# RKWin93/E2E-MAPPO-for-MT-FJSP

Hardware: NVIDIA B200
Metric: MT-FJSP env-steps/sec (higher is better)
Workload: dtype f64

## Files before the change

### e2e-mappo-for-mt-fjsp_b200/csrc/mtfjsp_gemm.cu

```cuda
#include <cuda.h>
#include <cuda_runtime.h>
#include <stdint.h>
#include <stdlib.h>

#include <type_traits>

#include "../../include/mtfjsp.h"

namespace {

constexpr int TILE_M = 128, TILE_N = 128;

__device__ __forceinline__ uint32_t smem_u32(const void* p) { return (uint32_t)__cvta_generic_to_shared(p); }
__device__ __forceinline__ float to_tf32(float x) {
    uint32_t r;
    asm("cvt.rna.tf32.f32 %0, %1;" : "=r"(r) : "f"(x));
    return __uint_as_float(r);
}
__device__ __forceinline__ void mbar_init(uint32_t bar, uint32_t count) {
    asm volatile("mbarrier.init.shared::cta.b64 [%0], %1;" ::"r"(bar), "r"(count));
}
__device__ __forceinline__ void mbar_wait(uint32_t bar, uint32_t parity) {
    uint32_t ok;
    do {
        asm volatile(
            "{\n\t.reg .pred p;\n\t"
            "mbarrier.try_wait.parity.shared::cta.b64 p, [%1], %2;\n\t"
            "selp.u32 %0, 1, 0, p;\n\t}"
            : "=r"(ok)
            : "r"(bar), "r"(parity)
            : "memory");
    } while (!ok);
}
__device__ __forceinline__ uint64_t make_desc(uint32_t saddr, uint32_t lbo_bytes, uint32_t sbo_bytes) {
    uint64_t d = 0;
    d |= (uint64_t)((saddr & 0x3FFFF) >> 4);
    d |= (uint64_t)(lbo_bytes >> 4) << 16;
    d |= (uint64_t)(sbo_bytes >> 4) << 32;
    d |= 1ull << 46;
    return d;
}
constexpr uint32_t IDESC = (1u << 4) | (2u << 7) | (2u << 10) | ((TILE_N >> 3) << 17) | ((TILE_M >> 4) << 24);

__device__ __forceinline__ void umma_tf32(uint32_t tmem_d, uint64_t adesc, uint64_t bdesc, uint32_t accumulate) {
    asm volatile(
        "{\n\t.reg .pred p;\n\tsetp.ne.b32 p, %4, 0;\n\t"
        "tcgen05.mma.cta_group::1.kind::tf32 [%0], %1, %2, %3, p;\n\t}" ::"r"(tmem_d),
        "l"(adesc), "l"(bdesc), "r"(IDESC), "r"(accumulate));
}

#define TMEM_LD32(taddr, r)                                                                                          \
    asm volatile(                                                                                                    \
        "tcgen05.ld.sync.aligned.32x32b.x32.b32 "                                                                    \
        "{%0,%1,%2,%3,%4,%5,%6,%7,%8,%9,%10,%11,%12,%13,%14,%15,%16,%17,%18,%19,%20,%21,%22,%23,%24,%25,%26,%27,%28,"  \
        "%29,%30,%31}, [%32];"                                                                                       \
        : "=r"(r[0]), "=r"(r[1]), "=r"(r[2]), "=r"(r[3]), "=r"(r[4]), "=r"(r[5]), "=r"(r[6]), "=r"(r[7]), "=r"(r[8]),  \
          "=r"(r[9]), "=r"(r[10]), "=r"(r[11]), "=r"(r[12]), "=r"(r[13]), "=r"(r[14]), "=r"(r[15]), "=r"(r[16]),       \
          "=r"(r[17]), "=r"(r[18]), "=r"(r[19]), "=r"(r[20]), "=r"(r[21]), "=r"(r[22]), "=r"(r[23]), "=r"(r[24]),      \
          "=r"(r[25]), "=r"(r[26]), "=r"(r[27]), "=r"(r[28]), "=r"(r[29]), "=r"(r[30]), "=r"(r[31])                    \
        : "r"(taddr))

template <bool AFFINE, int NWARPS>
__device__ __forceinline__ void stage_block(float* sdst, const float* __restrict__ g, long long row0, long long rows,
                                            int K, int KP, int ld, const float* s_scale, const float* s_shift,
                                            bool relu, int warp, int lane) {
    const int sbo = (KP / 4) * 128;
    const int r = lane & 7, c = lane >> 3;
    const int quads = KP / 16;
    const int total = 16 * quads;
    constexpr int U = 8;
    for (int it0 = warp; it0 < total; it0 += NWARPS * U) {
        float4 v[U];
#pragma unroll
        for (int u = 0; u < U; u++) {
            const int it = it0 + u * NWARPS;
            const int grp = it / quads, q = it - grp * quads;
            const long long row = row0 + grp * 8 + r;
            const int k = q * 16 + c * 4;
            v[u] = make_float4(0.f, 0.f, 0.f, 0.f);
            if (it < total && row < rows && k < K) v[u] = __ldg(reinterpret_cast<const float4*>(g + row * ld + k));
        }
#pragma unroll
        for (int u = 0; u < U; u++) {
            const int it = it0 + u * NWARPS;
            if (it >= total) break;
            const int grp = it / quads, q = it - grp * quads;
            const long long row = row0 + grp * 8 + r;
            const int k = q * 16 + c * 4;
            float4 x = v[u];
            if (AFFINE) {
                if (row < rows && k < K) {
                    x.x = x.x * s_scale[k] + s_shift[k]; x.y = x.y * s_scale[k + 1] + s_shift[k + 1];
                    x.z = x.z * s_scale[k + 2] + s_shift[k + 2]; x.w = x.w * s_scale[k + 3] + s_shift[k + 3];
                    if (relu) { x.x = fmaxf(x.x, 0.f); x.y = fmaxf(x.y, 0.f); x.z = fmaxf(x.z, 0.f); x.w = fmaxf(x.w, 0.f); }
                }
            }
            x.x = to_tf32(x.x); x.y = to_tf32(x.y); x.z = to_tf32(x.z); x.w = to_tf32(x.w);
            *reinterpret_cast<float4*>(reinterpret_cast<char*>(sdst) + grp * sbo + (q * 4 + c) * 128 + r * 16) = x;
        }
    }
}

constexpr int NPROD = 8;

template <int KS>
__device__ __forceinline__ void tile_issue(float* sdst, const float* __restrict__ g, long long row0, long long rows, int K,
                                           int kbase, int pw, int lane) {
    constexpr int SBO = (KS / 4) * 128, QUADS = KS / 16, TOTAL = 16 * QUADS;
    const int r = lane & 7, c = lane >> 3;
    static_assert(NPROD % QUADS == 0, "a warp keeps one K chunk: its folded BatchNorm constants live in registers");
#pragma unroll
    for (int it = pw; it < TOTAL; it += NPROD) {
        const int grp = it / QUADS, q = it % QUADS;
// ... 755 lines not shown
        for (int c = 0; c < nparts; c++) t += parts[((size_t)c * TILE_M + m) * NP + k];
        dW[idx] = t;
    }
    if (db && idx < TILE_M) {
        float t = 0.f;
        for (int c = 0; c < nparts; c++) t += dbparts[(size_t)c * 128 + idx];
        db[idx] = t;
    }
}


__device__ __forceinline__ float tanh_fast(float x) {
    const float t = __expf(2.f * fminf(x, 44.f));
    return 1.f - __fdividef(2.f, t + 1.f);
}
__device__ __forceinline__ float elu_fast(float x) { return x > 0.f ? x : __expf(x) - 1.f; }

constexpr int HEAD_WARPS = 16;

template <bool GROUPED>
__global__ void __launch_bounds__(HEAD_WARPS * 32, 1) head_tf32_kernel(
    const float* __restrict__ X, const int32_t* __restrict__ cand, long long rows, int rpe, int nodes_per_env,
    const float* __restrict__ in_scale, const float* __restrict__ in_shift, int in_relu, const float* __restrict__ Wa,
    const float* __restrict__ bias_env, long long bias_rows, const float* __restrict__ W1, const float* __restrict__ b1,
    const float* __restrict__ w2, const float* __restrict__ b2, float* __restrict__ out, long long num_tiles, int epg = 1) {
    extern __shared__ __align__(1024) unsigned char smem[];
    constexpr size_t WBYTES = (size_t)TILE_N * 128 * 4;
    float* sWa = reinterpret_cast<float*>(smem);
    float* sW1 = reinterpret_cast<float*>(smem + WBYTES);
    float* sA = reinterpret_cast<float*>(smem + 2 * WBYTES);
    float* s_part = reinterpret_cast<float*>(smem + 3 * WBYTES);
    float* s_b1 = s_part + 4 * 128;
    float* s_w2 = s_b1 + 128;
    float* s_scale = s_w2 + 128;
    float* s_shift = s_scale + 128;
    int* s_row = reinterpret_cast<int*>(s_shift + 128);
    uint64_t* s_bar = reinterpret_cast<uint64_t*>(s_row + 256);
    uint32_t* s_tmem = reinterpret_cast<uint32_t*>(s_bar + 2);

    const int tid = threadIdx.x, warp = tid >> 5, lane = tid & 31;
    const bool affine = in_scale != nullptr;
    if (tid < 128) {
        s_b1[tid] = b1 ? b1[tid] : 0.f;
        s_w2[tid] = w2[tid];
        s_scale[tid] = affine ? in_scale[tid] : 1.f;
        s_shift[tid] = affine ? in_shift[tid] : 0.f;
    }
    if (tid == 0) {
        mbar_init(smem_u32(s_bar + 0), 1);
        mbar_init(smem_u32(s_bar + 1), 1);
        asm volatile("fence.mbarrier_init.release.cluster;" ::: "memory");
    }
    if (warp == 0) {
        asm volatile("tcgen05.alloc.cta_group::1.sync.aligned.shared::cta.b32 [%0], %1;" ::"r"(smem_u32(s_tmem)), "r"(256));
        asm volatile("tcgen05.relinquish_alloc_permit.cta_group::1.sync.aligned;");
    }
    stage_block<false, HEAD_WARPS>(sWa, Wa, 0, TILE_N, 128, 128, 128, nullptr, nullptr, false, warp, lane);
    stage_block<false, HEAD_WARPS>(sW1, W1, 0, TILE_N, 128, 128, 128, nullptr, nullptr, false, warp, lane);
    auto fill_rows = [&](long long tile, int slot) {
        const long long r = tile * TILE_M + tid;
        int src = -1;
        if (tile < num_tiles && r < rows) src = cand ? (int)((r / rpe) * nodes_per_env + __ldg(cand + r)) : (int)r;
        s_row[slot * 128 + tid] = src;
    };
    if (tid < 128) fill_rows(blockIdx.x, 0);
    asm volatile("fence.proxy.async.shared::cta;" ::: "memory");
    asm volatile("tcgen05.fence::before_thread_sync;" ::: "memory");
    __syncthreads();
    asm volatile("tcgen05.fence::after_thread_sync;" ::: "memory");
    const uint32_t tmem_base = *s_tmem;
    const uint32_t bar0 = smem_u32(s_bar), bar1 = smem_u32(s_bar + 1);
    const float b2v = b2 ? __ldg(b2) : 0.f;

    const int r8 = lane & 7, c4 = lane >> 3;
    float4 v[8];
    auto gather = [&](int slot) {
#pragma unroll
        for (int u = 0; u < 8; u++) {
            const int it = warp + u * HEAD_WARPS, grp = it >> 3, q = it & 7;
            const int src = s_row[slot * 128 + grp * 8 + r8];
            v[u] = src >= 0 ? __ldg(reinterpret_cast<const float4*>(X + (size_t)src * 128 + q * 16 + c4 * 4)) : make_float4(0.f, 0.f, 0.f, 0.f);
        }
    };
    auto store_a = [&](int slot) {
#pragma unroll
        for (int u = 0; u < 8; u++) {
            const int it = warp + u * HEAD_WARPS, grp = it >> 3, q = it & 7, k = q * 16 + c4 * 4;
            float4 x = v[u];
            if (affine && s_row[slot * 128 + grp * 8 + r8] >= 0) {
                float4 sc, sh;
                if (GROUPED) {
                    const int src = s_row[slot * 128 + grp * 8 + r8];
                    const long long g = (long long)(cand ? src / nodes_per_env : src / rpe) / epg;
                    sc = __ldg(reinterpret_cast<const float4*>(in_scale + g * 128 + k));
                    sh = __ldg(reinterpret_cast<const float4*>(in_shift + g * 128 + k));
                } else {
                    sc = *reinterpret_cast<const float4*>(s_scale + k); sh = *reinterpret_cast<const float4*>(s_shift + k);
                }
                x.x = x.x * sc.x + sh.x; x.y = x.y * sc.y + sh.y; x.z = x.z * sc.z + sh.z; x.w = x.w * sc.w + sh.w;
                if (in_relu) { x.x = fmaxf(x.x, 0.f); x.y = fmaxf(x.y, 0.f); x.z = fmaxf(x.z, 0.f); x.w = fmaxf(x.w, 0.f); }
            }
            x.x = to_tf32(x.x); x.y = to_tf32(x.y); x.z = to_tf32(x.z); x.w = to_tf32(x.w);
            *reinterpret_cast<float4*>(reinterpret_cast<char*>(sA) + grp * 4096 + (q * 4 + c4) * 128 + r8 * 16) = x;
        }
    };
    auto mma_tile = [&](const float* sW, uint32_t dcol) {
        asm volatile("tcgen05.fence::after_thread_sync;" ::: "memory");
        const uint32_t aA = smem_u32(sA), aW = smem_u32(sW);
#pragma unroll
        for (int k = 0; k < 16; k++)
            umma_tf32(tmem_base + dcol, make_desc(aA + k * 256, 128, 4096), make_desc(aW + k * 256, 128, 4096), k > 0 ? 1u : 0u);
    };

    const int quad = warp & 3, cg = warp >> 2;
    const int trow = quad * 32 + lane;
    gather(0);
    long long i = 0;
    for (long long tile = blockIdx.x; tile < num_tiles; tile += gridDim.x, i++) {
        const int slot = (int)(i & 1);
        const uint32_t par = (uint32_t)(i & 1);
        store_a(slot);
        if (tid < 128) fill_rows(tile + gridDim.x, slot ^ 1);
        asm volatile("fence.proxy.async.shared::cta;" ::: "memory");
        asm volatile("tcgen05.fence::before_thread_sync;" ::: "memory");
        __syncthreads();
        if (tid == 0) {
            mma_tile(sWa, 0);
            asm volatile("tcgen05.commit.cta_group::1.mbarrier::arrive::one.shared::cluster.b64 [%0];" ::"r"(bar0) : "memory");
        }
        gather(slot ^ 1);
        mbar_wait(bar0, par);
        asm volatile("tcgen05.fence::after_thread_sync;" ::: "memory");
        const long long grow = tile * TILE_M + trow;
        const bool rok = grow < rows;
        {
            uint32_t r[32];
            TMEM_LD32(tmem_base + ((uint32_t)(quad * 32) << 16) + (uint32_t)(cg * 32), r);
            asm volatile("tcgen05.wait::ld.sync.aligned;" ::: "memory");
            const long long brow = bias_rows == 1 ? 0 : (rok ? grow / rpe : 0);
            const float4* bp = reinterpret_cast<const float4*>(bias_env + brow * 128 + cg * 32);
            char* dst = reinterpret_cast<char*>(sA) + (trow >> 3) * 4096 + (cg * 8) * 128 + (trow & 7) * 16;
#pragma unroll
            for (int j = 0; j < 8; j++) {
                const float4 bb = __ldg(bp + j);
                float4 x;
                x.x = to_tf32(tanh_fast(__uint_as_float(r[4 * j]) + bb.x)); x.y = to_tf32(tanh_fast(__uint_as_float(r[4 * j + 1]) + bb.y));
                x.z = to_tf32(tanh_fast(__uint_as_float(r[4 * j + 2]) + bb.z)); x.w = to_tf32(tanh_fast(__uint_as_float(r[4 * j + 3]) + bb.w));
                if (!rok) x = make_float4(0.f, 0.f, 0.f, 0.f);
                *reinterpret_cast<float4*>(dst + j * 128) = x;
            }
        }
        asm volatile("fence.proxy.async.shared::cta;" ::: "memory");
        asm volatile("tcgen05.fence::before_thread_sync;" ::: "memory");
        __syncthreads();
        if (tid == 0) {
            mma_tile(sW1, TILE_N);
            asm volatile("tcgen05.commit.cta_group::1.mbarrier::arrive::one.shared::cluster.b64 [%0];" ::"r"(bar1) : "memory");
        }
        mbar_wait(bar1, par);
        asm volatile("tcgen05.fence::after_thread_sync;" ::: "memory");
        {
            uint32_t r[32];
            TMEM_LD32(tmem_base + ((uint32_t)(quad * 32) << 16) + (uint32_t)(TILE_N + cg * 32), r);
            asm volatile("tcgen05.wait::ld.sync.aligned;" ::: "memory");
            float acc = 0.f;
#pragma unroll
            for (int j = 0; j < 8; j++) {
                const float4 bb = *reinterpret_cast<const float4*>(s_b1 + cg * 32 + 4 * j);
                const float4 ww = *reinterpret_cast<const float4*>(s_w2 + cg * 32 + 4 * j);
                acc = fmaf(tanh_fast(__uint_as_float(r[4 * j]) + bb.x), ww.x, acc);
                acc = fmaf(tanh_fast(__uint_as_float(r[4 * j + 1]) + bb.y), ww.y, acc);
                acc = fmaf(tanh_fast(__uint_as_float(r[4 * j + 2]) + bb.z), ww.z, acc);
                acc = fmaf(tanh_fast(__uint_as_float(r[4 * j + 3]) + bb.w), ww.w, acc);
            }
            s_part[cg * 128 + trow] = acc;
        }
        asm volatile("tcgen05.fence::before_thread_sync;" ::: "memory");
        __syncthreads();
        if (tid < 128) {
            const long long orow = tile * TILE_M + tid;
            if (orow < rows) out[orow] = ((s_part[tid] + s_part[128 + tid]) + (s_part[256 + tid] + s_part[384 + tid])) + b2v;
        }
    }
    asm volatile("tcgen05.fence::before_thread_sync;" ::: "memory");
    __syncthreads();
    if (warp == 0) asm volatile("tcgen05.dealloc.cta_group::1.sync.aligned.b32 %0, %1;" ::"r"(tmem_base), "r"(256));
}


constexpr int TRUNK_WARPS = 16;
template <bool GROUPED>
__global__ void __launch_bounds__(TRUNK_WARPS * 32, 1) gat_trunk2_tf32_kernel(
    const float* __restrict__ f1, const float* __restrict__ f2, const float* __restrict__ W1p, const float* __restrict__ W2p,
    const float* __restrict__ Wt, const float* __restrict__ a_src, const float* __restrict__ a_dst, float* __restrict__ out,
    double* __restrict__ stats, long long R, long long num_tiles, int rpt, int M) {
    extern __shared__ __align__(1024) unsigned char smem[];
    constexpr size_t WBYTES = (size_t)TILE_N * 128 * 4;
    float* sW = reinterpret_cast<float*>(smem);
    float* sA1 = reinterpret_cast<float*>(smem + WBYTES);
    float* sA2 = reinterpret_cast<float*>(smem + 2 * WBYTES);
    float* s_dot = reinterpret_cast<float*>(smem + 3 * WBYTES);
    float* s_as = s_dot + 3 * 4 * 128;
    float* s_ad = s_as + 128;
    float* s_w1p = s_ad + 128;
    float* s_w2p = s_w1p + 128 * 6;
    uint64_t* s_bar = reinterpret_cast<uint64_t*>(s_w2p + 128 * 8);
    uint32_t* s_tmem = reinterpret_cast<uint32_t*>(s_bar + 1);

    const int tid = threadIdx.x, warp = tid >> 5, lane = tid & 31;
    if (tid < 128) { s_as[tid] = a_src[tid]; s_ad[tid] = a_dst[tid]; }
    for (int i = tid; i < 128 * 6; i += blockDim.x) s_w1p[i] = W1p[i];
    for (int i = tid; i < 128 * 8; i += blockDim.x) s_w2p[i] = W2p[i];
    if (tid == 0) {
        mbar_init(smem_u32(s_bar), 1);
        asm volatile("fence.mbarrier_init.release.cluster;" ::: "memory");
    }
    if (warp == 0) {
        asm volatile("tcgen05.alloc.cta_group::1.sync.aligned.shared::cta.b32 [%0], %1;" ::"r"(smem_u32(s_tmem)), "r"(256));
        asm volatile("tcgen05.relinquish_alloc_permit.cta_group::1.sync.aligned;");
    }
    stage_block<false, TRUNK_WARPS>(sW, Wt, 0, TILE_N, 128, 128, 128, nullptr, nullptr, false, warp, lane);
    asm volatile("fence.proxy.async.shared::cta;" ::: "memory");
    asm volatile("tcgen05.fence::before_thread_sync;" ::: "memory");
    __syncthreads();
    asm volatile("tcgen05.fence::after_thread_sync;" ::: "memory");
    const uint32_t tmem_base = *s_tmem;
    const uint32_t bar = smem_u32(s_bar);

    const int quad = warp & 3, cg = warp >> 2;
    const int mloc = quad * 32 + lane;
    const size_t arow = (size_t)(mloc >> 3) * 4096 + (cg * 8) * 128 + (mloc & 7) * 16;
    uint32_t phase = 0;
    double st_sum = 0.0, st_sq = 0.0;
    for (long long tile = blockIdx.x; tile < num_tiles; tile += gridDim.x) {
        const long long m = tile * (GROUPED ? rpt : 128) + mloc;
        const bool mok = m < R && (!GROUPED || mloc < rpt);
        {
            float fa[6] = {0.f, 0.f, 0.f, 0.f, 0.f, 0.f}, fb[8] = {0.f, 0.f, 0.f, 0.f, 0.f, 0.f, 0.f, 0.f};
            if (mok) {
                const float2* p2 = reinterpret_cast<const float2*>(f1 + m * 6);
                const float2 u0 = __ldg(p2), u1 = __ldg(p2 + 1), u2 = __ldg(p2 + 2);
                fa[0] = u0.x; fa[1] = u0.y; fa[2] = u1.x; fa[3] = u1.y; fa[4] = u2.x; fa[5] = u2.y;
                const float4 v0 = __ldg(reinterpret_cast<const float4*>(f2 + m * 8)), v1 = __ldg(reinterpret_cast<const float4*>(f2 + m * 8) + 1);
                fb[0] = v0.x; fb[1] = v0.y; fb[2] = v0.z; fb[3] = v0.w; fb[4] = v1.x; fb[5] = v1.y; fb[6] = v1.z; fb[7] = v1.w;
            }
#pragma unroll
            for (int j = 0; j < 8; j++) {
                float o1[4], o2[4];
// ... 23 lines not shown
                for (int k = 0; k < 16; k++)
                    umma_tf32(tmem_base, make_desc(a1 + k * 256, 128, 4096), make_desc(aW + k * 256, 128, 4096), k > 0 ? 1u : 0u);
#pragma unroll
                for (int k = 0; k < 16; k++)
                    umma_tf32(tmem_base + TILE_N, make_desc(a2 + k * 256, 128, 4096), make_desc(aW + k * 256, 128, 4096), k > 0 ? 1u : 0u);
                asm volatile("tcgen05.commit.cta_group::1.mbarrier::arrive::one.shared::cluster.b64 [%0];" ::"r"(bar) : "memory");
            }
            mbar_wait(bar, phase);
            phase ^= 1;
            asm volatile("tcgen05.fence::after_thread_sync;" ::: "memory");
            uint32_t r1[32], r2[32];
            TMEM_LD32(tmem_base + ((uint32_t)(quad * 32) << 16) + (uint32_t)(cg * 32), r1);
            TMEM_LD32(tmem_base + ((uint32_t)(quad * 32) << 16) + (uint32_t)(TILE_N + cg * 32), r2);
            asm volatile("tcgen05.wait::ld.sync.aligned;" ::: "memory");
            float ps = 0.f, pd1 = 0.f, pd2 = 0.f;
#pragma unroll
            for (int j = 0; j < 8; j++) {
                const float4 va = *reinterpret_cast<const float4*>(s_as + cg * 32 + 4 * j), vd = *reinterpret_cast<const float4*>(s_ad + cg * 32 + 4 * j);
                const float x0 = __uint_as_float(r1[4 * j]), x1 = __uint_as_float(r1[4 * j + 1]), x2 = __uint_as_float(r1[4 * j + 2]),
                            x3 = __uint_as_float(r1[4 * j + 3]);
                const float y0 = __uint_as_float(r2[4 * j]), y1 = __uint_as_float(r2[4 * j + 1]), y2 = __uint_as_float(r2[4 * j + 2]),
                            y3 = __uint_as_float(r2[4 * j + 3]);
                ps = fmaf(x3, va.w, fmaf(x2, va.z, fmaf(x1, va.y, fmaf(x0, va.x, ps))));
                pd1 = fmaf(x3, vd.w, fmaf(x2, vd.z, fmaf(x1, vd.y, fmaf(x0, vd.x, pd1))));
                pd2 = fmaf(y3, vd.w, fmaf(y2, vd.z, fmaf(y1, vd.y, fmaf(y0, vd.x, pd2))));
            }
            s_dot[(0 * 4 + cg) * 128 + mloc] = ps;
            s_dot[(1 * 4 + cg) * 128 + mloc] = pd1;
            s_dot[(2 * 4 + cg) * 128 + mloc] = pd2;
            asm volatile("tcgen05.fence::before_thread_sync;" ::: "memory");
            __syncthreads();
            const float s1 = (s_dot[0 * 128 + mloc] + s_dot[1 * 128 + mloc]) + (s_dot[2 * 128 + mloc] + s_dot[3 * 128 + mloc]);
            const float d1 = (s_dot[4 * 128 + mloc] + s_dot[5 * 128 + mloc]) + (s_dot[6 * 128 + mloc] + s_dot[7 * 128 + mloc]);
            const float d2 = (s_dot[8 * 128 + mloc] + s_dot[9 * 128 + mloc]) + (s_dot[10 * 128 + mloc] + s_dot[11 * 128 + mloc]);
            float e11 = s1 + d1, e12 = s1 + d2;
            e11 = e11 > 0.f ? e11 : 0.2f * e11;
            e12 = e12 > 0.f ? e12 : 0.2f * e12;
            const float mx = fmaxf(e11, e12);
            const float p1 = expf(e11 - mx), p2 = expf(e12 - mx);
            const float a0 = p1 / (p1 + p2), a1 = p2 / (p1 + p2);
            if (layer < 2) {
#pragma unroll
                for (int j = 0; j < 8; j++) {
                    float4 x, y;
                    y.x = __uint_as_float(r2[4 * j]); y.y = __uint_as_float(r2[4 * j + 1]); y.z = __uint_as_float(r2[4 * j + 2]); y.w = __uint_as_float(r2[4 * j + 3]);
                    x.x = a0 * __uint_as_float(r1[4 * j]) + a1 * y.x; x.y = a0 * __uint_as_float(r1[4 * j + 1]) + a1 * y.y;
                    x.z = a0 * __uint_as_float(r1[4 * j + 2]) + a1 * y.z; x.w = a0 * __uint_as_float(r1[4 * j + 3]) + a1 * y.w;
                    x.x = to_tf32(elu_fast(x.x)); x.y = to_tf32(elu_fast(x.y)); x.z = to_tf32(elu_fast(x.z)); x.w = to_tf32(elu_fast(x.w));
                    y.x = to_tf32(elu_fast(y.x)); y.y = to_tf32(elu_fast(y.y)); y.z = to_tf32(elu_fast(y.z)); y.w = to_tf32(elu_fast(y.w));
                    *reinterpret_cast<float4*>(reinterpret_cast<char*>(sA1) + arow + j * 128) = x;
                    *reinterpret_cast<float4*>(reinterpret_cast<char*>(sA2) + arow + j * 128) = y;
                }
            } else {
                float4* op = reinterpret_cast<float4*>(out + m * 128 + cg * 32);
                float o[32];
#pragma unroll
                for (int j = 0; j < 32; j++) {
                    const float y = __uint_as_float(r2[j]);
                    o[j] = mok ? 0.5f * ((a0 * __uint_as_float(r1[j]) + a1 * y) + y) : 0.f;
                }
                if (mok) {
#pragma unroll
                    for (int j = 0; j < 8; j++) op[j] = make_float4(o[4 * j], o[4 * j + 1], o[4 * j + 2], o[4 * j + 3]);
                }
                if (GROUPED) {
#pragma unroll
                    for (int j = 0; j < 8; j++)
                        *reinterpret_cast<float4*>(sA1 + mloc * 128 + (((cg * 8 + j) ^ (mloc & 7)) << 2)) =
                            make_float4(o[4 * j], o[4 * j + 1], o[4 * j + 2], o[4 * j + 3]);
                }
                if (!GROUPED && stats) {
                    float q[32];
#pragma unroll
                    for (int j = 0; j < 32; j++) q[j] = o[j] * o[j];
#pragma unroll
                    for (int off = 16, n = 16; off >= 1; off >>= 1, n >>= 1) {
                        const bool up = (lane & off) != 0;
#pragma unroll
                        for (int j = 0; j < n; j++) {
                            const float so = up ? o[j] : o[j + n], ko = up ? o[j + n] : o[j];
                            const float sq = up ? q[j] : q[j + n], kq = up ? q[j + n] : q[j];
                            o[j] = ko + __shfl_xor_sync(0xffffffffu, so, off);
                            q[j] = kq + __shfl_xor_sync(0xffffffffu, sq, off);
                        }
                    }
                    st_sum += (double)o[0];
                    st_sq += (double)q[0];
                }
            }
        }
        __syncthreads();
        if (GROUPED) {
            const long long row0 = tile * rpt, env0 = row0 / M;
            const int nenv = (int)(R - row0 < rpt ? R - row0 : rpt) / M;
            for (int item = tid; item < nenv * 128; item += TRUNK_WARPS * 32) {
                const int e = item >> 7, c = item & 127;
                double sum = 0.0, sq = 0.0;
                for (int j = 0; j < M; j++) {
                    const int r = e * M + j;
                    const double v = (double)sA1[r * 128 + ((((c >> 2) ^ (r & 7))) << 2) + (c & 3)];
                    sum += v;
                    sq = fma(v, v, sq);
                }
                stats[(env0 + e) * 256 + c] = sum;
                stats[(env0 + e) * 256 + 128 + c] = sq;
            }
            __syncthreads();
        }
    }
    if (!GROUPED && stats) {
        atomicAdd(stats + cg * 32 + lane, st_sum);
        atomicAdd(stats + 128 + cg * 32 + lane, st_sq);
    }
    asm volatile("tcgen05.fence::before_thread_sync;" ::: "memory");
    __syncthreads();
    if (warp == 0) asm volatile("tcgen05.dealloc.cta_group::1.sync.aligned.b32 %0, %1;" ::"r"(tmem_base), "r"(256));
}


constexpr int ESA_MOMENTS = 14 + 36 + 64, ESA_STATS_THREADS = 256, ESA_STATS_ROWS = 256, ESA_STATS_BLOCKS = 592;

__global__ void __launch_bounds__(ESA_STATS_THREADS) esa_stats_kernel(const float* __restrict__ f1, const float* __restrict__ f2,
                                                                       long long B, int M, int epc, double* __restrict__ parts,
                                                                       float* __restrict__ env_mean) {
    __shared__ float s_f[ESA_STATS_ROWS * 14];
    __shared__ double s_acc[128];
    const int tid = threadIdx.x, mom = tid & 127, half = tid >> 7;
    int ca = 0, cb = -1;
    if (mom < 14) ca = mom;
    else if (mom < 50) { ca = (mom - 14) / 6; cb = (mom - 14) % 6; }
    else if (mom < ESA_MOMENTS) { ca = 6 + (mom - 50) / 8; cb = 6 + (mom - 50) % 8; }
    double acc = 0.0;
    const long long chunks = (B + epc - 1) / epc;
    for (long long ch = blockIdx.x; ch < chunks; ch += gridDim.x) {
        const long long e0 = ch * epc;
        const int ne = (int)(B - e0 < epc ? B - e0 : epc), nr = ne * M;
        const long long r0 = e0 * M;
        __syncthreads();
        for (int i = tid; i < nr * 6; i += ESA_STATS_THREADS) s_f[(i / 6) * 14 + i % 6] = __ldg(f1 + r0 * 6 + i);
        for (int i = tid; i < nr * 8; i += ESA_STATS_THREADS) s_f[(i / 8) * 14 + 6 + i % 8] = __ldg(f2 + r0 * 8 + i);
        __syncthreads();
        if (mom < ESA_MOMENTS) {
            if (cb < 0) {
                for (int r = half; r < nr; r += 2) acc += (double)s_f[r * 14 + ca];
            } else {
                for (int r = half; r < nr; r += 2) acc = fma((double)s_f[r * 14 + ca], (double)s_f[r * 14 + cb], acc);
            }
        }
        for (int i = tid; i < ne * 16; i += ESA_STATS_THREADS) {
            const int e = i >> 4, c = i & 15;
            double s = 0.0;
            if (c < 14)
                for (int m = 0; m < M; m++) s += (double)s_f[(e * M + m) * 14 + c];
            env_mean[(e0 + e) * 16 + c] = (float)(s / M);
        }
    }
    if (half == 1) s_acc[mom] = acc;
    __syncthreads();
    if (half == 0) parts[(size_t)blockIdx.x * 128 + mom] = acc + s_acc[mom];
}

__global__ void esa_stats_reduce_kernel(const double* __restrict__ parts, int nparts, double* __restrict__ moments) {
// ... 334 lines not shown
    else
        linear_tf32_tma_kernel<false, true><<<grid, GEMM_WARPS * 32, smem_lin, stream>>>(
            map, rows, W, bias, in_scale, in_shift, in_relu, Z, env_stats, tiles, rpt, N, nullptr, nullptr, P, epg);
    return cudaGetLastError() == cudaSuccess ? 1 : MTFJSP_E_CUDA;
}

extern "C" {

int mtfjsp_enc_linear_tf32(const float* X, int64_t rows, int K, const float* W, const float* bias, const float* in_scale,
                           const float* in_shift, int in_relu, float* Z, double* stats, void* stream) {
    if (!X || !W || !Z || rows < 1 || K < 4 || K > 128 || (K % 4) != 0) return MTFJSP_E_ARG;
    if ((in_scale == nullptr) != (in_shift == nullptr)) return MTFJSP_E_ARG;
    if (!al16(X, W, Z) || !al8(stats)) return MTFJSP_E_ARG;
    cudaStream_t s = (cudaStream_t)stream;
    if (K == 128 && rows >= 4096) {
        const int rc = launch_linear_tma(X, rows, W, bias, in_scale, in_shift, in_relu, Z, stats, s);
        if (rc != 0) return rc < 0 ? rc : MTFJSP_OK;
    }
    if (K <= 16) return launch_linear<16>(X, rows, K, W, bias, in_scale, in_shift, in_relu, Z, stats, s);
    if (K <= 32) return launch_linear<32>(X, rows, K, W, bias, in_scale, in_shift, in_relu, Z, stats, s);
    if (K <= 64) return launch_linear<64>(X, rows, K, W, bias, in_scale, in_shift, in_relu, Z, stats, s);
    return launch_linear<128>(X, rows, K, W, bias, in_scale, in_shift, in_relu, Z, stats, s);
}

int mtfjsp_enc_head_tf32(const float* X, const int32_t* cand, int64_t B, int rows_per_env, int nodes_per_env,
                         const float* in_scale, const float* in_shift, int in_relu, const float* Wa, const float* bias_env,
                         int64_t bias_rows, const float* W1, const float* b1, const float* w2, const float* b2, float* out,
                         void* stream) {
    if (!X || !Wa || !bias_env || !W1 || !w2 || !out || B < 1 || rows_per_env < 1) return MTFJSP_E_ARG;
    if ((in_scale == nullptr) != (in_shift == nullptr)) return MTFJSP_E_ARG;
    if (!al16(X, Wa, bias_env, W1)) return MTFJSP_E_ARG;
    if (bias_rows != 1 && bias_rows != B) return MTFJSP_E_ARG;
    if (cand && (nodes_per_env < 1 || (long long)B * nodes_per_env > 0x7fffffffLL)) return MTFJSP_E_ARG;
    const long long rows = (long long)B * rows_per_env;
    if (rows > 0x7fffffffLL) return MTFJSP_E_ARG;
    const size_t smem = 3 * (size_t)TILE_N * 128 * 4 + (4 * 128 + 4 * 128) * 4 + 256 * 4 + 2 * 8 + 16;
    static thread_local bool configured = false;
    if (!configured) {
        if (cudaFuncSetAttribute(head_tf32_kernel<false>, cudaFuncAttributeMaxDynamicSharedMemorySize, (int)smem) != cudaSuccess)
            return MTFJSP_E_CUDA;
        configured = true;
    }
    int dev = 0, sms = 148;
    cudaGetDevice(&dev);
    cudaDeviceGetAttribute(&sms, cudaDevAttrMultiProcessorCount, dev);
    const long long tiles = (rows + TILE_M - 1) / TILE_M;
    const int grid = (int)(tiles < sms ? tiles : sms);
    head_tf32_kernel<false><<<grid, HEAD_WARPS * 32, smem, (cudaStream_t)stream>>>(X, cand, rows, rows_per_env, nodes_per_env, in_scale,
                                                                          in_shift, in_relu, Wa, bias_env, bias_rows, W1, b1, w2, b2,
                                                                          out, tiles);
    return cudaGetLastError() == cudaSuccess ? MTFJSP_OK : MTFJSP_E_CUDA;
}

int mtfjsp_enc_gat_trunk_tf32(const float* fea1, const float* fea2, const float* W1p, const float* W2p, const float* Wt,
                              const float* a_src, const float* a_dst, float* out, double* stats, int64_t R, void* stream) {
    if (!fea1 || !fea2 || !W1p || !W2p || !Wt || !a_src || !a_dst || !out || R < 1) return MTFJSP_E_ARG;
    if (!al16(fea2, Wt, out) || !al8(fea1) || !al8(stats)) return MTFJSP_E_ARG;
    const size_t smem = 3 * (size_t)TILE_N * 128 * 4 + (3 * 4 * 128 + 256 + 128 * 14) * 4 + 8 + 16;
    static thread_local bool configured = false;
    if (!configured) {
        if (cudaFuncSetAttribute(gat_trunk2_tf32_kernel<false>, cudaFuncAttributeMaxDynamicSharedMemorySize, (int)smem) != cudaSuccess)
            return MTFJSP_E_CUDA;
        configured = true;
    }
    int dev = 0, sms = 148;
    cudaGetDevice(&dev);
    cudaDeviceGetAttribute(&sms, cudaDevAttrMultiProcessorCount, dev);
    const long long tiles = (R + 127) / 128;
    const int grid = (int)(tiles < sms ? tiles : sms);
    gat_trunk2_tf32_kernel<false><<<grid, TRUNK_WARPS * 32, smem, (cudaStream_t)stream>>>(fea1, fea2, W1p, W2p, Wt, a_src, a_dst, out,
                                                                                          stats, R, tiles, 128, 1);
    return cudaGetLastError() == cudaSuccess ? MTFJSP_OK : MTFJSP_E_CUDA;
}

int mtfjsp_enc_gat_trunk_tf32_grouped(const float* fea1, const float* fea2, const float* W1p, const float* W2p, const float* Wt,
                                      const float* a_src, const float* a_dst, float* out, double* env_stats, int64_t B, int M,
                                      void* stream) {
    if (!fea1 || !fea2 || !W1p || !W2p || !Wt || !a_src || !a_dst || !out || !env_stats || B < 1 || M < 1 || M > 128 ||
        B * M > 0x7fffff00LL)
        return MTFJSP_E_ARG;
    if (!al16(fea2, Wt, out) || !al8(fea1) || !al8(env_stats)) return MTFJSP_E_ARG;
    const size_t smem = 3 * (size_t)TILE_N * 128 * 4 + (3 * 4 * 128 + 256 + 128 * 14) * 4 + 8 + 16;
    static thread_local bool configured = false;
    if (!configured) {
        if (cudaFuncSetAttribute(gat_trunk2_tf32_kernel<true>, cudaFuncAttributeMaxDynamicSharedMemorySize, (int)smem) != cudaSuccess)
            return MTFJSP_E_CUDA;
        configured = true;
    }
    int dev = 0, sms = 148;
    cudaGetDevice(&dev);
    cudaDeviceGetAttribute(&sms, cudaDevAttrMultiProcessorCount, dev);
    const int epT = 128 / M;
    const long long tiles = (B + epT - 1) / epT;
    const int grid = (int)(tiles < sms ? tiles : sms);
    gat_trunk2_tf32_kernel<true><<<grid, TRUNK_WARPS * 32, smem, (cudaStream_t)stream>>>(fea1, fea2, W1p, W2p, Wt, a_src, a_dst, out,
                                                                                         env_stats, B * M, tiles, epT * M, M);
    return cudaGetLastError() == cudaSuccess ? MTFJSP_OK : MTFJSP_E_CUDA;
}

int mtfjsp_enc_aggregate_linear_tf32(const float* X, int64_t B, int N, const float* adj_w, const int16_t* adj_src, const float* W,
                                     const float* bias, const float* in_scale, const float* in_shift, int in_relu, float* Z,
                                     double* stats, void* stream) {
    if (!X || !adj_w || !adj_src || !W || !Z || B < 1 || N < 1) return MTFJSP_E_ARG;
    if ((in_scale == nullptr) != (in_shift == nullptr)) return MTFJSP_E_ARG;
    if (!al16(X, W, Z) || !al8(adj_w) || !al8(stats)) return MTFJSP_E_ARG;
    const int rc = launch_linear_tma_agg(X, B, N, adj_w, adj_src, W, bias, in_scale, in_shift, in_relu, Z, stats, (cudaStream_t)stream);
    if (rc == 0) return MTFJSP_E_STATE;
    return rc < 0 ? rc : MTFJSP_OK;
}

static bool grouped_args_ok(int64_t B, int N, int epg) { return B >= 1 && N >= 1 && epg >= 1 && B % epg == 0 && B * N <= 0x7fffff00LL; }

int mtfjsp_enc_linear_tf32_grouped(const float* X, int64_t B, int rows_per_env, int K, const float* W, const float* bias,
                                   const float* in_scale, const float* in_shift, int in_relu, int envs_per_group, float* Z,
                                   double* env_stats, void* stream) {
    if (!X || !W || !Z || !env_stats || !grouped_args_ok(B, rows_per_env, envs_per_group)) return MTFJSP_E_ARG;
    if ((in_scale == nullptr) != (in_shift == nullptr)) return MTFJSP_E_ARG;
    if (!al16(X, W, Z, in_scale, in_shift) || !al8(env_stats)) return MTFJSP_E_ARG;
    if (K == 128) {
        const int rc = launch_linear_tma_grouped(false, X, B, rows_per_env, nullptr, nullptr, W, bias, in_scale, in_shift, in_relu,
                                                 envs_per_group, Z, env_stats, (cudaStream_t)stream);
        return rc == 0 ? MTFJSP_E_STATE : rc < 0 ? rc : MTFJSP_OK;
    }
    if (K < 4 || K > 16 || (K % 4) != 0 || in_scale) return MTFJSP_E_ARG;
    return launch_linear<16, true>(X, B * rows_per_env, K, W, bias, nullptr, nullptr, 0, Z, env_stats, (cudaStream_t)stream, rows_per_env);
}

int mtfjsp_enc_aggregate_linear_tf32_grouped(const float* X, int64_t B, int N, const float* adj_w, const int16_t* adj_src,
                                             const float* W, const float* bias, const float* in_scale, const float* in_shift,
                                             int in_relu, int envs_per_group, float* Z, double* env_stats, void* stream) {
    if (!X || !adj_w || !adj_src || !W || !Z || !env_stats || !grouped_args_ok(B, N, envs_per_group)) return MTFJSP_E_ARG;
    if ((in_scale == nullptr) != (in_shift == nullptr)) return MTFJSP_E_ARG;
    if (!al16(X, W, Z, in_scale, in_shift) || !al8(adj_w) || !al8(env_stats)) return MTFJSP_E_ARG;
    if (N > TILE_M) return MTFJSP_E_STATE;
    const int rc = launch_linear_tma_grouped(true, X, B, N, adj_w, adj_src, W, bias, in_scale, in_shift, in_relu, envs_per_group, Z,
                                             env_stats, (cudaStream_t)stream);
    return rc == 0 ? MTFJSP_E_STATE : rc < 0 ? rc : MTFJSP_OK;
}

int mtfjsp_enc_head_tf32_grouped(const float* X, const int32_t* cand, int64_t B, int rows_per_env, int nodes_per_env,
                                 const float* in_scale, const float* in_shift, int in_relu, int envs_per_group, const float* Wa,
                                 const float* bias_env, int64_t bias_rows, const float* W1, const float* b1, const float* w2,
                                 const float* b2, float* out, void* stream) {
    if (!X || !in_scale || !in_shift || !Wa || !bias_env || !W1 || !w2 || !out || B < 1 || rows_per_env < 1) return MTFJSP_E_ARG;
    if (envs_per_group < 1 || B % envs_per_group != 0) return MTFJSP_E_ARG;
    if (bias_rows != 1 && bias_rows != B) return MTFJSP_E_ARG;
    if (!al16(X, Wa, bias_env, W1, in_scale, in_shift)) return MTFJSP_E_ARG;
    if (cand && (nodes_per_env < 1 || (long long)B * nodes_per_env > 0x7fffffffLL)) return MTFJSP_E_ARG;
// ... 136 lines not shown
```

Baseline: 1.072 billion.

## Pipeline head MMAs via TMEM A-operand and TMA-store trunk outputs

The head kernel now writes the tanh intermediate back into tensor memory and issues the second MMA with A read from TMEM instead of shared memory. It also issues the next tile's first MMA before waiting on the current second MMA, so the two GEMM stages overlap; this needs 512 TMEM columns. The trunk kernel stages its output in swizzled shared memory and writes it with bulk tensor (TMA) stores instead of per-thread global stores. This adds a tensor-map encode on every host call and an extra wait on the bulk store each iteration. A profiling script is added as well.

```diff
diff --git a/e2e-mappo-for-mt-fjsp_b200/csrc/mtfjsp_gemm.cu b/e2e-mappo-for-mt-fjsp_b200/csrc/mtfjsp_gemm.cu
--- a/e2e-mappo-for-mt-fjsp_b200/csrc/mtfjsp_gemm.cu
+++ b/e2e-mappo-for-mt-fjsp_b200/csrc/mtfjsp_gemm.cu
@@ -59,6 +59,23 @@
           "=r"(r[17]), "=r"(r[18]), "=r"(r[19]), "=r"(r[20]), "=r"(r[21]), "=r"(r[22]), "=r"(r[23]), "=r"(r[24]),      \
           "=r"(r[25]), "=r"(r[26]), "=r"(r[27]), "=r"(r[28]), "=r"(r[29]), "=r"(r[30]), "=r"(r[31])                    \
         : "r"(taddr))
+
+#define TMEM_ST32(taddr, r)                                                                                          \
+    asm volatile(                                                                                                    \
+        "tcgen05.st.sync.aligned.32x32b.x32.b32 [%0], "                                                              \
+        "{%1,%2,%3,%4,%5,%6,%7,%8,%9,%10,%11,%12,%13,%14,%15,%16,%17,%18,%19,%20,%21,%22,%23,%24,%25,%26,%27,%28,%29," \
+        "%30,%31,%32};" ::"r"(taddr),                                                                                  \
+        "r"(r[0]), "r"(r[1]), "r"(r[2]), "r"(r[3]), "r"(r[4]), "r"(r[5]), "r"(r[6]), "r"(r[7]), "r"(r[8]), "r"(r[9]),     \
+        "r"(r[10]), "r"(r[11]), "r"(r[12]), "r"(r[13]), "r"(r[14]), "r"(r[15]), "r"(r[16]), "r"(r[17]), "r"(r[18]),       \
+        "r"(r[19]), "r"(r[20]), "r"(r[21]), "r"(r[22]), "r"(r[23]), "r"(r[24]), "r"(r[25]), "r"(r[26]), "r"(r[27]),       \
+        "r"(r[28]), "r"(r[29]), "r"(r[30]), "r"(r[31]) : "memory")
+
+__device__ __forceinline__ void umma_tf32_tmem_a(uint32_t tmem_d, uint32_t tmem_a, uint64_t bdesc, uint32_t accumulate) {
+    asm volatile(
+        "{\n\t.reg .pred p;\n\tsetp.ne.b32 p, %4, 0;\n\t"
+        "tcgen05.mma.cta_group::1.kind::tf32 [%0], [%1], %2, %3, p;\n\t}" ::"r"(tmem_d),
+        "r"(tmem_a), "l"(bdesc), "r"(IDESC), "r"(accumulate));
+}
 
 template <bool AFFINE, int NWARPS>
 __device__ __forceinline__ void stage_block(float* sdst, const float* __restrict__ g, long long row0, long long rows,
@@ -920,7 +937,7 @@
         asm volatile("fence.mbarrier_init.release.cluster;" ::: "memory");
     }
     if (warp == 0) {
-        asm volatile("tcgen05.alloc.cta_group::1.sync.aligned.shared::cta.b32 [%0], %1;" ::"r"(smem_u32(s_tmem)), "r"(256));
+        asm volatile("tcgen05.alloc.cta_group::1.sync.aligned.shared::cta.b32 [%0], %1;" ::"r"(smem_u32(s_tmem)), "r"(512));
         asm volatile("tcgen05.relinquish_alloc_permit.cta_group::1.sync.aligned;");
     }
     stage_block<false, HEAD_WARPS>(sWa, Wa, 0, TILE_N, 128, 128, 128, nullptr, nullptr, false, warp, lane);
@@ -982,13 +999,9 @@
 
     const int quad = warp & 3, cg = warp >> 2;
     const int trow = quad * 32 + lane;
-    gather(0);
-    long long i = 0;
-    for (long long tile = blockIdx.x; tile < num_tiles; tile += gridDim.x, i++) {
-        const int slot = (int)(i & 1);
-        const uint32_t par = (uint32_t)(i & 1);
+    auto issue_first = [&](int slot, long long next) {
         store_a(slot);
-        if (tid < 128) fill_rows(tile + gridDim.x, slot ^ 1);
+        if (tid < 128) fill_rows(next, slot ^ 1);
         asm volatile("fence.proxy.async.shared::cta;" ::: "memory");
         asm volatile("tcgen05.fence::before_thread_sync;" ::: "memory");
         __syncthreads();
@@ -997,6 +1010,13 @@
             asm volatile("tcgen05.commit.cta_group::1.mbarrier::arrive::one.shared::cluster.b64 [%0];" ::"r"(bar0) : "memory");
         }
         gather(slot ^ 1);
+    };
+    gather(0);
+    if ((long long)blockIdx.x < num_tiles) issue_first(0, (long long)blockIdx.x + gridDim.x);
+    long long i = 0;
+    for (long long tile = blockIdx.x; tile < num_tiles; tile += gridDim.x, i++) {
+        const int slot = (int)(i & 1);
+        const uint32_t par = (uint32_t)(i & 1);
         mbar_wait(bar0, par);
         asm volatile("tcgen05.fence::after_thread_sync;" ::: "memory");
         const long long grow = tile * TILE_M + trow;
@@ -1007,7 +1027,6 @@
             asm volatile("tcgen05.wait::ld.sync.aligned;" ::: "memory");
             const long long brow = bias_rows == 1 ? 0 : (rok ? grow / rpe : 0);
             const float4* bp = reinterpret_cast<const float4*>(bias_env + brow * 128 + cg * 32);
-            char* dst = reinterpret_cast<char*>(sA) + (trow >> 3) * 4096 + (cg * 8) * 128 + (trow & 7) * 16;
 #pragma unroll
             for (int j = 0; j < 8; j++) {
                 const float4 bb = __ldg(bp + j);
@@ -1015,16 +1034,22 @@
                 x.x = to_tf32(tanh_fast(__uint_as_float(r[4 * j]) + bb.x)); x.y = to_tf32(tanh_fast(__uint_as_float(r[4 * j + 1]) + bb.y));
                 x.z = to_tf32(tanh_fast(__uint_as_float(r[4 * j + 2]) + bb.z)); x.w = to_tf32(tanh_fast(__uint_as_float(r[4 * j + 3]) + bb.w));
                 if (!rok) x = make_float4(0.f, 0.f, 0.f, 0.f);
-                *reinterpret_cast<float4*>(dst + j * 128) = x;
-            }
-        }
-        asm volatile("fence.proxy.async.shared::cta;" ::: "memory");
+                r[4 * j] = __float_as_uint(x.x); r[4 * j + 1] = __float_as_uint(x.y); r[4 * j + 2] = __float_as_uint(x.z); r[4 * j + 3] = __float_as_uint(x.w);
+            }
+            TMEM_ST32(tmem_base + ((uint32_t)(quad * 32) << 16) + (uint32_t)(2 * TILE_N + cg * 32), r);
+            asm volatile("tcgen05.wait::st.sync.aligned;" ::: "memory");
+        }
         asm volatile("tcgen05.fence::before_thread_sync;" ::: "memory");
         __syncthreads();
         if (tid == 0) {
-            mma_tile(sW1, TILE_N);
+            asm volatile("tcgen05.fence::after_thread_sync;" ::: "memory");
+            const uint32_t aW = smem_u32(sW1);
+#pragma unroll
+            for (int k = 0; k < 16; k++)
+                umma_tf32_tmem_a(tmem_base + TILE_N, tmem_base + 2 * TILE_N + k * 8, make_desc(aW + k * 256, 128, 4096), k > 0 ? 1u : 0u);
             asm volatile("tcgen05.commit.cta_group::1.mbarrier::arrive::one.shared::cluster.b64 [%0];" ::"r"(bar1) : "memory");
         }
+        if (tile + gridDim.x < num_tiles) issue_first(slot ^ 1, tile + 2 * (long long)gridDim.x);
         mbar_wait(bar1, par);
         asm volatile("tcgen05.fence::after_thread_sync;" ::: "memory");
         {
@@ -1052,7 +1077,7 @@
     }
     asm volatile("tcgen05.fence::before_thread_sync;" ::: "memory");
     __syncthreads();
-    if (warp == 0) asm volatile("tcgen05.dealloc.cta_group::1.sync.aligned.b32 %0, %1;" ::"r"(tmem_base), "r"(256));
+    if (warp == 0) asm volatile("tcgen05.dealloc.cta_group::1.sync.aligned.b32 %0, %1;" ::"r"(tmem_base), "r"(512));
 }
 
 
@@ -1060,8 +1085,8 @@
 template <bool GROUPED>
 __global__ void __launch_bounds__(TRUNK_WARPS * 32, 1) gat_trunk2_tf32_kernel(
     const float* __restrict__ f1, const float* __restrict__ f2, const float* __restrict__ W1p, const float* __restrict__ W2p,
-    const float* __restrict__ Wt, const float* __restrict__ a_src, const float* __restrict__ a_dst, float* __restrict__ out,
-    double* __restrict__ stats, long long R, long long num_tiles, int rpt, int M) {
+    const float* __restrict__ Wt, const float* __restrict__ a_src, const float* __restrict__ a_dst,
+    const __grid_constant__ CUtensorMap tmapOut, double* __restrict__ stats, long long R, long long num_tiles, int rpt, int M) {
     extern __shared__ __align__(1024) unsigned char smem[];
     constexpr size_t WBYTES = (size_t)TILE_N * 128 * 4;
     float* sW = reinterpret_cast<float*>(smem);
@@ -1191,23 +1216,16 @@
                     *reinterpret_cast<float4*>(reinterpret_cast<char*>(sA2) + arow + j * 128) = y;
                 }
             } else {
-                float4* op = reinterpret_cast<float4*>(out + m * 128 + cg * 32);
                 float o[32];
 #pragma unroll
                 for (int j = 0; j < 32; j++) {
                     const float y = __uint_as_float(r2[j]);
                     o[j] = mok ? 0.5f * ((a0 * __uint_as_float(r1[j]) + a1 * y) + y) : 0.f;
                 }
-                if (mok) {
-#pragma unroll
-                    for (int j = 0; j < 8; j++) op[j] = make_float4(o[4 * j], o[4 * j + 1], o[4 * j + 2], o[4 * j + 3]);
-                }
-                if (GROUPED) {
-#pragma unroll
-                    for (int j = 0; j < 8; j++)
-                        *reinterpret_cast<float4*>(sA1 + mloc * 128 + (((cg * 8 + j) ^ (mloc & 7)) << 2)) =
-                            make_float4(o[4 * j], o[4 * j + 1], o[4 * j + 2], o[4 * j + 3]);
-                }
+#pragma unroll
+                for (int j = 0; j < 8; j++)
+                    *reinterpret_cast<float4*>(sA1 + cg * 4096 + mloc * 32 + ((j ^ (mloc & 7)) << 2)) =
+                        make_float4(o[4 * j], o[4 * j + 1], o[4 * j + 2], o[4 * j + 3]);
                 if (!GROUPED && stats) {
                     float q[32];
 #pragma unroll
@@ -1228,25 +1246,37 @@
                 }
             }
         }
+        const long long row0 = tile * (GROUPED ? rpt : 128);
+        asm volatile("fence.proxy.async.shared::cta;" ::: "memory");
         __syncthreads();
+        if (tid == 0) {
+#pragma unroll
+            for (int c = 0; c < 4; c++)
+                asm volatile("cp.async.bulk.tensor.2d.global.shared::cta.bulk_group [%0, {%1, %2}], [%3];" ::"l"(&tmapOut), "r"(c * 32),
+                             "r"((int)row0), "r"(smem_u32(sA1 + c * 4096))
+                             : "memory");
+            asm volatile("cp.async.bulk.commit_group;" ::: "memory");
+        }
         if (GROUPED) {
-            const long long row0 = tile * rpt, env0 = row0 / M;
+            const long long env0 = row0 / M;
             const int nenv = (int)(R - row0 < rpt ? R - row0 : rpt) / M;
             for (int item = tid; item < nenv * 128; item += TRUNK_WARPS * 32) {
                 const int e = item >> 7, c = item & 127;
                 double sum = 0.0, sq = 0.0;
                 for (int j = 0; j < M; j++) {
                     const int r = e * M + j;
-                    const double v = (double)sA1[r * 128 + ((((c >> 2) ^ (r & 7))) << 2) + (c & 3)];
+                    const double v = (double)sA1[(c >> 5) * 4096 + r * 32 + ((((c >> 2) & 7) ^ (r & 7)) << 2) + (c & 3)];
                     sum += v;
                     sq = fma(v, v, sq);
                 }
                 stats[(env0 + e) * 256 + c] = sum;
                 stats[(env0 + e) * 256 + 128 + c] = sq;
             }
-            __syncthreads();
-        }
-    }
+        }
+        if (tid == 0) asm volatile("cp.async.bulk.wait_group.read 0;" ::: "memory");
+        __syncthreads();
+    }
+    if (tid == 0) asm volatile("cp.async.bulk.wait_group 0;" ::: "memory");
     if (!GROUPED && stats) {
         atomicAdd(stats + cg * 32 + lane, st_sum);
         atomicAdd(stats + 128 + cg * 32 + lane, st_sq);
@@ -1687,6 +1717,17 @@
     return cudaGetLastError() == cudaSuccess ? MTFJSP_OK : MTFJSP_E_CUDA;
 }
 
+static bool trunk_out_map(CUtensorMap* map, float* out, long long R, int rpt) {
+    EncodeTiledFn enc = encode_tiled_fn();
+    if (!enc) return false;
+    const cuuint64_t dims[2] = {128, (cuuint64_t)R};
+    const cuuint64_t strides[1] = {512};
+    const cuuint32_t box[2] = {32, (cuuint32_t)rpt};
+    const cuuint32_t estr[2] = {1, 1};
+    return enc(map, CU_TENSOR_MAP_DATA_TYPE_FLOAT32, 2, (void*)out, dims, strides, box, estr, CU_TENSOR_MAP_INTERLEAVE_NONE,
+               CU_TENSOR_MAP_SWIZZLE_128B, CU_TENSOR_MAP_L2_PROMOTION_NONE, CU_TENSOR_MAP_FLOAT_OOB_FILL_NONE) == CUDA_SUCCESS;
+}
+
 int mtfjsp_enc_gat_trunk_tf32(const float* fea1, const float* fea2, const float* W1p, const float* W2p, const float* Wt,
                               const float* a_src, const float* a_dst, float* out, double* stats, int64_t R, void* stream) {
     if (!fea1 || !fea2 || !W1p || !W2p || !Wt || !a_src || !a_dst || !out || R < 1) return MTFJSP_E_ARG;
@@ -1703,7 +1744,9 @@
     cudaDeviceGetAttribute(&sms, cudaDevAttrMultiProcessorCount, dev);
     const long long tiles = (R + 127) / 128;
     const int grid = (int)(tiles < sms ? tiles : sms);
-    gat_trunk2_tf32_kernel<false><<<grid, TRUNK_WARPS * 32, smem, (cudaStream_t)stream>>>(fea1, fea2, W1p, W2p, Wt, a_src, a_dst, out,
+    CUtensorMap map;
+    if (!trunk_out_map(&map, out, R, 128)) return MTFJSP_E_CUDA;
+    gat_trunk2_tf32_kernel<false><<<grid, TRUNK_WARPS * 32, smem, (cudaStream_t)stream>>>(fea1, fea2, W1p, W2p, Wt, a_src, a_dst, map,
                                                                                           stats, R, tiles, 128, 1);
     return cudaGetLastError() == cudaSuccess ? MTFJSP_OK : MTFJSP_E_CUDA;
 }
@@ -1728,7 +1771,9 @@
     const int epT = 128 / M;
     const long long tiles = (B + epT - 1) / epT;
     const int grid = (int)(tiles < sms ? tiles : sms);
-    gat_trunk2_tf32_kernel<true><<<grid, TRUNK_WARPS * 32, smem, (cudaStream_t)stream>>>(fea1, fea2, W1p, W2p, Wt, a_src, a_dst, out,
+    CUtensorMap map;
+    if (!trunk_out_map(&map, out, B * M, epT * M)) return MTFJSP_E_CUDA;
+    gat_trunk2_tf32_kernel<true><<<grid, TRUNK_WARPS * 32, smem, (cudaStream_t)stream>>>(fea1, fea2, W1p, W2p, Wt, a_src, a_dst, map,
                                                                                          env_stats, B * M, tiles, epT * M, M);
     return cudaGetLastError() == cudaSuccess ? MTFJSP_OK : MTFJSP_E_CUDA;
 }
diff --git a/profiles/prof_heads_trunk.py b/profiles/prof_heads_trunk.py
--- /dev/null
+++ b/profiles/prof_heads_trunk.py
@@ -0,0 +1,176 @@
+import argparse
+import importlib
+import json
+import os
+import subprocess
+import sys
+
+sys.path.insert(0, os.path.dirname(os.path.dirname(os.path.abspath(__file__))))
+import torch
+
+PKG = "e2e-mappo-for-mt-fjsp_b200"
+libm = importlib.import_module(PKG + "._lib")
+enc = importlib.import_module(PKG + ".encoder")
+
+
+def card():
+    q = "name,power.limit,clocks.sm,clocks.max.sm"
+    try:
+        return subprocess.run(["nvidia-smi", "--query-gpu=" + q, "--format=csv,noheader"], capture_output=True, text=True,
+                              timeout=30).stdout.strip().splitlines()[0]
+    except Exception as e:
+        return "unread (%s)" % e
+
+
+def use_lib(path):
+    libm._lib = None
+    libm.LIB_PATH = path
+    libm.lib()
+
+
+def cases(dev):
+    g = torch.Generator(device="cpu").manual_seed(5)
+
+    def rnd(*shape, scale=1.0):
+        return (torch.randn(*shape, generator=g) * scale).to(dev)
+
+    out = {}
+    B, M = 65536, 6
+    R = B * M
+    f1, f2 = rnd(R, 6), rnd(R, 8)
+    W1p, W2p, Wt = rnd(128, 6, scale=0.3), rnd(128, 8, scale=0.3), rnd(128, 128, scale=0.09)
+    a_src, a_dst = rnd(128, scale=0.1), rnd(128, scale=0.1)
+    stats = torch.zeros(256, dtype=torch.float64, device=dev)
+    env_stats = torch.empty((B, 1, 2, 128), dtype=torch.float64, device=dev)
+
+    def trunk_g1():
+        stats.zero_()
+        return enc.gat_trunk_tf32(f1, f2, W1p, W2p, Wt, a_src, a_dst, stats), stats
+
+    def trunk_g4096():
+        return enc.gat_trunk_tf32_grouped(f1, f2, W1p, W2p, Wt, a_src, a_dst, env_stats, M), env_stats
+
+    out["trunk_g1"] = (trunk_g1, 2.0 * R * 128 * 128 * 6)
+    out["trunk_g4096"] = (trunk_g4096, 2.0 * R * 128 * 128 * 6)
+
+    Wa, W1 = rnd(128, 128, scale=0.09), rnd(128, 128, scale=0.09)
+    b1, w2, b2 = rnd(128, scale=0.1), rnd(128, scale=0.09), rnd(1, scale=0.1)
+    sc, sh = (1.0 + rnd(128, scale=0.1)), rnd(128, scale=0.1)
+    xm, bias_m = rnd(R, 128), rnd(B, 128, scale=0.3)
+    out["mhead_J6M6"] = (lambda: (enc.head_tf32(xm, None, B, M, 0, sc, sh, Wa, bias_m, W1, b1, w2, b2, relu=False),),
+                         2.0 * R * 128 * 128 * 2)
+    for (J, Mj, Bj) in ((6, 6, 65536), (10, 10, 16384), (30, 20, 4096)):
+        N = J * Mj
+        xj = rnd(Bj, N, 128)
+        cand = torch.randint(0, N, (Bj, J), generator=g, dtype=torch.int32).to(dev)
+        bias_j = rnd(Bj, 128, scale=0.3)
+        out["jhead_J%dM%d" % (J, Mj)] = (
+            lambda xj=xj, cand=cand, bias_j=bias_j, Bj=Bj, J=J, N=N:
+            (enc.head_tf32(xj, cand, Bj, J, N, sc, sh, Wa, bias_j, W1, b1, w2, b2, relu=True),),
+            2.0 * Bj * J * 128 * 128 * 2)
+    return out
+
+
+def rollout_table(steps=4):
+    pkg = importlib.import_module(PKG)
+    envm = importlib.import_module(PKG + ".env")
+    rom = importlib.import_module(PKG + ".rollout")
+    from torch.profiler import ProfilerActivity, profile
+    B, J, M, E = 65536, 6, 6, 2
+    d = pkg.instances.synthetic_instances(0, B, J, M, E, 1002)
+    env = envm.BatchedMTFJSPEnv(B, J, M, E, obs_dtype=torch.float32)
+    env.load(d["t"], d["p"], d["transT"], d["edge"])
+    env.scaler_init()
+    job = enc.JobActor(enc.seeded_state_dict(enc.job_actor_keys(128), 11), J, M, precision="tf32")
+    mch = enc.MachineActor(enc.seeded_state_dict(enc.machine_actor_keys(128), 12), M, precision="tf32")
+    ro = rom.Rollout(env, job, mch, greedy=False, use_cuda_graph=False, seed=1)
+    ro.begin_episode(pkg.instances.random_weights(0, B, 1002))
+    for _ in range(4):
+        ro.step()
+    torch.cuda.synchronize()
+    with profile(activities=[ProfilerActivity.CUDA]) as prof:
+        for _ in range(steps):
+            ro.step()
+        torch.cuda.synchronize()
+    rows = []
+    for ev in prof.key_averages():
+        t = getattr(ev, "device_time_total", None)
+        if t is None:
+            t = ev.cuda_time_total
+        if t > 0:
+            rows.append((t / steps, ev.count / steps, ev.key))
+    rows.sort(reverse=True)
+    return {"steps": steps, "us_per_step_total": sum(r[0] for r in rows),
+            "kernels": [{"us_per_step": round(t, 1), "launches_per_step": c, "name": k[:120]} for t, c, k in rows[:25]]}
+
+
+def main():
+    ap = argparse.ArgumentParser()
+    ap.add_argument("--lib", action="append", default=[], help="NAME=PATH of a libmtfjsp_b200.so build (default: in-tree)")
+    ap.add_argument("--reps", type=int, default=40)
+    ap.add_argument("--rounds", type=int, default=3)
+    ap.add_argument("--out", default=None)
+    ap.add_argument("--rollout-table", action="store_true")
+    args = ap.parse_args()
+    libs = [tuple(s.split("=", 1)) for s in args.lib] or [("tree", libm.LIB_PATH)]
+    dev = torch.device("cuda", 0)
+    torch.cuda.set_device(dev)
+    flush = torch.empty(256 << 20, dtype=torch.uint8, device=dev)
+    cs = cases(dev)
+    res = {"card": card(), "reps_per_round": args.reps, "rounds": args.rounds, "l2": "256 MB memset before each call",
+           "ms": {n: {c: [] for c in cs} for n, _ in libs}, "max_abs_diff_vs_first": {}}
+    first = {}
+    with torch.no_grad():
+        for n, p in libs:
+            use_lib(p)
+            for c, (fn, _) in cs.items():
+                for _ in range(3):
+                    o = fn()
+                torch.cuda.synchronize()
+                o = [t.clone() for t in o]
+                if not first.get(c):
+                    first[c] = o
+                else:
+                    res["max_abs_diff_vs_first"].setdefault(n, {})[c] = {
+                        "bitwise_equal": all(torch.equal(a, b) for a, b in zip(first[c], o)),
+                        "max_abs": max(float((a.double() - b.double()).abs().max()) for a, b in zip(first[c], o))}
+        e0, e1 = torch.cuda.Event(enable_timing=True), torch.cuda.Event(enable_timing=True)
+        for _ in range(args.rounds):
+            for n, p in libs:
+                use_lib(p)
+                for c, (fn, _) in cs.items():
+                    for _ in range(args.reps):
+                        flush.zero_()
+                        e0.record()
+                        fn()
+                        e1.record()
+                        e1.synchronize()
+                        res["ms"][n][c].append(e0.elapsed_time(e1))
+    summ = {}
+    for n, _ in libs:
+        summ[n] = {}
+        for c, (_, flops) in cs.items():
+            v = sorted(res["ms"][n][c])
+            med = v[len(v) // 2]
+            per_round = [sorted(res["ms"][n][c][r * args.reps:(r + 1) * args.reps])[args.reps // 2] for r in range(args.rounds)]
+            summ[n][c] = {"median_us": round(med * 1e3, 1), "round_medians_us": [round(x * 1e3, 1) for x in per_round],
+                          "tf32_tflops": round(flops / (med * 1e-3) / 1e12, 1)}
+        t = summ[n]
+        summ[n]["rollout_trunk_plus_heads_us"] = round(t["trunk_g1"]["median_us"] + t["mhead_J6M6"]["median_us"] +
+                                                       t["jhead_J6M6"]["median_us"], 1)
+    res["summary"] = summ
+    del res["ms"]
+    if args.rollout_table:
+        use_lib(libs[0][1])
+        res["rollout_step_kernels"] = rollout_table()
+    res["card_after"] = card()
+    txt = json.dumps(res, indent=1)
+    print(txt)
+    if args.out:
+        os.makedirs(os.path.dirname(os.path.abspath(args.out)), exist_ok=True)
+        with open(args.out, "w") as f:
+            f.write(txt + "\n")
+
+
+if __name__ == "__main__":
+    main()
```

New measurement: 1.072 billion, median of 6. No clear change (-0.1%).
